# daxiongpro/EPNet

Measured on AMD Instinct MI355X. Metric: SA-stack points/sec per GPU (16384-pt KITTI scene) + % HBM roofline, higher is better.
Workload: dtype f32; 1 GPU; 256 x 16384-pt kitti scenes per GPU per step through the 4-level SA op stack (4 samplings [FPS + centre gather; levels 2-4 nested in level 1 where tie-free] + 8 ball_query + 8 fused groupings [xyz - centre ; features]), pyramid 16384>4096>1024>256>64, radii [[.1,.5],[.5,1],[1,2],[2,4]], nsample [16,32], C=0/96/256/512, HIP-graph launch; levels=4, scenes_per_gpu=256, software_pipelined=True, pipeline_stages=2, parallelism=scene-parallel x1

## Files before the change

epnet_amd/csrc/ball_query.hip:

```cpp

#include "common.h"
#include "dpp.h"
#include "spatial.h"

namespace epnet {

constexpr int kBqTile = 2048;
constexpr int kBqThreads = 256;

template <int CPW>
__global__ __launch_bounds__(kBqThreads) void ball_query_kernel(int n, int m, float radius2, int nsample,
                                                                const float *__restrict__ new_xyz,
                                                                const float *__restrict__ xyz,
                                                                int *__restrict__ idx) {
    __shared__ float tile[kBqTile * 3];
    const int lane = threadIdx.x & 63, wave = threadIdx.x >> 6;
    const int bs = blockIdx.y;
    xyz += (size_t)bs * n * 3;
    new_xyz += (size_t)bs * m * 3;
    idx += (size_t)bs * m * nsample;

    const int c0 = (blockIdx.x * (kBqThreads / 64) + wave) * CPW;
    float cx[CPW], cy[CPW], cz[CPW];
    int cnt[CPW], first[CPW];
#pragma unroll
    for (int i = 0; i < CPW; ++i) {
        const int ci = c0 + i;
        const bool ok = ci < m;
        cx[i] = ok ? new_xyz[ci * 3 + 0] : 0.f;
        cy[i] = ok ? new_xyz[ci * 3 + 1] : 0.f;
        cz[i] = ok ? new_xyz[ci * 3 + 2] : 0.f;
        cnt[i] = ok ? 0 : nsample;
        first[i] = 0;
    }

    for (int t0 = 0; t0 < n; t0 += kBqTile) {
        const int tn = min(kBqTile, n - t0);
        for (int e = threadIdx.x; e < tn * 3; e += kBqThreads) tile[e] = xyz[(size_t)t0 * 3 + e];
        __syncthreads();

        bool wave_done = true;
#pragma unroll
        for (int i = 0; i < CPW; ++i) wave_done = wave_done && (cnt[i] >= nsample);

        if (!wave_done) {
            for (int p0 = 0; p0 < tn; p0 += 64) {
                const int p = p0 + lane;
                const bool valid = p < tn;
                const float x = valid ? tile[p * 3 + 0] : 0.f;
                const float y = valid ? tile[p * 3 + 1] : 0.f;
                const float z = valid ? tile[p * 3 + 2] : 0.f;
                bool all_full = true;
#pragma unroll
                for (int i = 0; i < CPW; ++i) {
                    if (cnt[i] < nsample) {
                        const float dx = cx[i] - x, dy = cy[i] - y, dz = cz[i] - z;
                        const float d2 = dx * dx + dy * dy + dz * dz;
                        const bool hit = valid && (d2 < radius2);
                        const unsigned long long mask = __ballot(hit);
                        if (mask) {
                            const int pos = cnt[i] + popc_below(mask);
                            if (hit && pos < nsample) idx[(size_t)(c0 + i) * nsample + pos] = t0 + p;
                            if (cnt[i] == 0) first[i] = t0 + p0 + (int)__builtin_ctzll(mask);
                            cnt[i] += (int)__popcll(mask);
                        }
                        all_full = all_full && (cnt[i] >= nsample);
                    }
                }
                if (all_full) {
                    wave_done = true;
                    break;
                }
            }
        }
        if (__syncthreads_and(wave_done ? 1 : 0)) break;
    }

#pragma unroll
    for (int i = 0; i < CPW; ++i) {
        const int ci = c0 + i;
        if (ci < m && cnt[i] < nsample) {
            const int fill = cnt[i] > 0 ? first[i] : 0;
            for (int l = cnt[i] + lane; l < nsample; l += 64) idx[(size_t)ci * nsample + l] = fill;
        }
    }
}



#ifdef EPNET_BQ_STATS
__device__ unsigned long long g_bq_stats[16];
#endif
#ifdef EPNET_IX_STATS
__device__ unsigned long long g_ix_stats[8];
#define EPNET_IX_STAMP(var) const unsigned long long var = __builtin_amdgcn_s_memtime()
#else
#define EPNET_IX_STAMP(var)
#endif

template <int kIxThreads, int BITS>
__global__ __launch_bounds__(kIxThreads) void bq_index_kernel(int n, int np, const float *__restrict__ xyz,
                                                              float4 *__restrict__ sorted, float *__restrict__ boxes,
                                                              float *__restrict__ qboxes, int n_src = 0,
                                                              const int *__restrict__ src_idx = nullptr,
                                                              float *__restrict__ gathered = nullptr) {
    constexpr int kCells = 1 << BITS;
    extern __shared__ int s_hist[];
    __shared__ float s_box[6][16];
    __shared__ int s_part[16];
    const int q = threadIdx.x, lane = q & 63, wave = q >> 6;
    __builtin_amdgcn_s_setprio(3);
    xyz += (size_t)blockIdx.x * (src_idx ? n_src : n) * 3;
    if (src_idx) {
        src_idx += (size_t)blockIdx.x * n;
        gathered += (size_t)blockIdx.x * n * 3;
    }
    sorted += (size_t)blockIdx.x * np;
    boxes += (size_t)blockIdx.x * (np / 64) * 6;
    constexpr int per = kCells / kIxThreads;
    constexpr int per_shift = per == 16 ? 4 : per == 8 ? 3 : per == 4 ? 2 : -1;
    static_assert(per_shift > 0, "scan layout");
    constexpr int kIxPerThread = 16;
    const bool in_regs = n <= kIxThreads * kIxPerThread;
    float px[kIxPerThread], py[kIxPerThread], pz[kIxPerThread];
    float lo[3], ext[3];
    EPNET_IX_STAMP(t_0);
    if (in_regs) {
        float mn[3] = {3.4e38f, 3.4e38f, 3.4e38f}, mx[3] = {-3.4e38f, -3.4e38f, -3.4e38f};
        int row[kIxPerThread];
#pragma unroll
        for (int i = 0; i < kIxPerThread; ++i) {
            const int k = q + i * kIxThreads;
            const int kk = k < n ? k : 0;
            row[i] = src_idx ? src_idx[kk] : kk;
        }
#pragma unroll
        for (int i = 0; i < kIxPerThread; ++i) {
            px[i] = xyz[row[i] * 3 + 0];
            py[i] = xyz[row[i] * 3 + 1];
            pz[i] = xyz[row[i] * 3 + 2];
        }
        if (src_idx) {
#pragma unroll
            for (int i = 0; i < kIxPerThread; ++i) {
                const int k = q + i * kIxThreads;
                if (k < n) {
                    gathered[k * 3 + 0] = px[i];
                    gathered[k * 3 + 1] = py[i];
                    gathered[k * 3 + 2] = pz[i];
                }
            }
        }
#pragma unroll
        for (int i = 0; i < kIxPerThread; ++i) {
            const bool ok = q + i * kIxThreads < n;
            mn[0] = fminf(mn[0], ok ? px[i] : 3.4e38f); mx[0] = fmaxf(mx[0], ok ? px[i] : -3.4e38f);
            mn[1] = fminf(mn[1], ok ? py[i] : 3.4e38f); mx[1] = fmaxf(mx[1], ok ? py[i] : -3.4e38f);
            mn[2] = fminf(mn[2], ok ? pz[i] : 3.4e38f); mx[2] = fmaxf(mx[2], ok ? pz[i] : -3.4e38f);
        }
#pragma unroll
        for (int a = 0; a < 3; ++a) {
            const float l = wave_minf_all(mn[a]), h = wave_maxf_all(mx[a]);
            if (lane == 0) {
                s_box[a][wave] = l;
                s_box[3 + a][wave] = h;
            }
        }
        __syncthreads();
#pragma unroll
        for (int a = 0; a < 3; ++a) {
            float l = s_box[a][0], h = s_box[3 + a][0];
            for (int w = 1; w < kIxThreads / 64; ++w) {
                l = fminf(l, s_box[a][w]);
                h = fmaxf(h, s_box[3 + a][w]);
            }
            lo[a] = l;
            ext[a] = h - l;
        }
    } else {
        block_bbox3(xyz, n, s_box, lo, ext);
    }
    const CellGrid g = make_cell_grid(lo, ext, BITS);
    EPNET_IX_STAMP(t_1);
    for (int i = q; i < kCells + kCells / per + 64; i += kIxThreads) s_hist[i] = 0;
    __syncthreads();
    EPNET_IX_STAMP(t_2);
    int code[kIxPerThread], rank[kIxPerThread];
    if (in_regs) {
#pragma unroll
        for (int i = 0; i < kIxPerThread; ++i) code[i] = hist_at((int)cell_code(g, px[i], py[i], pz[i]), per_shift);
#pragma unroll
        for (int i = 0; i < kIxPerThread; ++i)
            rank[i] = atomicAdd(&s_hist[q + i * kIxThreads < n ? code[i] : kCells + kCells / per + lane], 1);
    } else {
        for (int k = q; k < n; k += kIxThreads)
            atomicAdd(&s_hist[hist_at((int)cell_code(g, xyz[k * 3 + 0], xyz[k * 3 + 1], xyz[k * 3 + 2]), per_shift)], 1);
    }
    __syncthreads();
    EPNET_IX_STAMP(t_3);
    int sum = 0;
    for (int i = 0; i < per; ++i) sum += s_hist[hist_at(q * per + i, per_shift)];
    const int incl = wave_inclusive_scan(sum);
    if (lane == 63) s_part[wave] = incl;
    __syncthreads();
    int base = incl - sum;
    for (int w = 0; w < wave; ++w) base += s_part[w];
    for (int i = 0; i < per; ++i) {
        const int at = hist_at(q * per + i, per_shift);
        const int c = s_hist[at];
        s_hist[at] = base;
        base += c;
    }
    __syncthreads();
    EPNET_IX_STAMP(t_4);
    auto bucket_box = [&](int p, const float4 v) {
        const bool real = p < n;
        const float cx_ = canonical(v.x), cy_ = canonical(v.y), cz_ = canonical(v.z);
        float mnx = real ? cx_ : 3.4e38f, mxx = real ? cx_ : -3.4e38f, mny = real ? cy_ : 3.4e38f, mxy = real ? cy_ : -3.4e38f,
              mnz = real ? cz_ : 3.4e38f, mxz = real ? cz_ : -3.4e38f;
        wave_box(mnx, mxx, mny, mxy, mnz, mxz);
        if (lane == 0) {
            float *bx = boxes + (p >> 6) * 6;
            const bool any = mnx <= mxx;
            bx[0] = any ? mnx : 3.0e38f; bx[1] = any ? mxx : 3.0e38f;
            bx[2] = any ? mny : 3.0e38f; bx[3] = any ? mxy : 3.0e38f;
            bx[4] = any ? mnz : 3.0e38f; bx[5] = any ? mxz : 3.0e38f;
        }
    };
    const bool staged = in_regs && (np & 255) == 0;
    if (staged) {
        float4 *s_stage = reinterpret_cast<float4 *>(s_hist + kCells + kCells / per + 64);
        int pos[kIxPerThread];
#pragma unroll
        for (int i = 0; i < kIxPerThread; ++i) pos[i] = s_hist[code[i]] + rank[i];
        const int quarter = kIxThreads == 256 ? min(np >> 2, 512) : np >> 2;
        for (int h = 0; h * quarter < np; ++h) {
            const int base = h * quarter, len = min(quarter, np - base);
            for (int p = q; p < len; p += kIxThreads)
                if (base + p >= n) s_stage[p] = make_float4(3.0e38f, 3.0e38f, 3.0e38f, __int_as_float(-1));
#pragma unroll
            for (int i = 0; i < kIxPerThread; ++i) {
                const int k = q + i * kIxThreads;
                if (k < n && (unsigned)(pos[i] - base) < (unsigned)quarter)
                    s_stage[pos[i] - base] = make_float4(px[i], py[i], pz[i], __int_as_float(k));
            }
            __syncthreads();
            for (int p = q; p < len; p += kIxThreads) {
                const float4 v = s_stage[p];
                sorted[base + p] = v;
                bucket_box(base + p, v);
            }
            __syncthreads();
        }
    } else {
        if (in_regs) {
#pragma unroll
            for (int i = 0; i < kIxPerThread; ++i) {
                const int k = q + i * kIxThreads;
                if (k < n) sorted[s_hist[code[i]] + rank[i]] = make_float4(px[i], py[i], pz[i], __int_as_float(k));
            }
        } else {
            for (int k = q; k < n; k += kIxThreads) {
                const float x = xyz[k * 3 + 0], y = xyz[k * 3 + 1], z = xyz[k * 3 + 2];
                const int pos = atomicAdd(&s_hist[hist_at((int)cell_code(g, x, y, z), per_shift)], 1);
                sorted[pos] = make_float4(x, y, z, __int_as_float(k));
            }
        }
        for (int p = n + q; p < np; p += kIxThreads)
            sorted[p] = make_float4(3.0e38f, 3.0e38f, 3.0e38f, __int_as_float(-1));
        __threadfence_block();
        __syncthreads();
        for (int p = q; p < np; p += kIxThreads) bucket_box(p, sorted[p]);
    }
#ifdef EPNET_IX_STATS
    {
        EPNET_IX_STAMP(t_6);
        if (q == 0) {
            atomicAdd(&g_ix_stats[0], t_1 - t_0); atomicAdd(&g_ix_stats[1], t_2 - t_1); atomicAdd(&g_ix_stats[2], t_3 - t_2);
            atomicAdd(&g_ix_stats[3], t_4 - t_3); atomicAdd(&g_ix_stats[4], t_6 - t_4);
            atomicAdd(&g_ix_stats[7], 1ull);
        }
    }
#endif
    if (!qboxes) return;
    qboxes += (size_t)blockIdx.x * (np / 256) * 6;
    __threadfence_block();
    __syncthreads();
    for (int g = q; g < np / 256; g += kIxThreads) {
        float mn[3] = {3.4e38f, 3.4e38f, 3.4e38f}, mx[3] = {-3.4e38f, -3.4e38f, -3.4e38f};
        for (int k = 0; k < 4; ++k) {
            const float *bx = boxes + (g * 4 + k) * 6;
            if (bx[0] < 3.0e38f)
#pragma unroll
                for (int a = 0; a < 3; ++a) {
                    mn[a] = fminf(mn[a], bx[2 * a]);
                    mx[a] = fmaxf(mx[a], bx[2 * a + 1]);
                }
        }
        const bool any = mn[0] <= mx[0];
#pragma unroll
        for (int a = 0; a < 3; ++a) {
            qboxes[g * 6 + 2 * a] = any ? mn[a] : 3.0e38f;
            qboxes[g * 6 + 2 * a + 1] = any ? mx[a] : 3.0e38f;
        }
    }
}

constexpr int kQThreads = 256;

__device__ __forceinline__ bool box_near(const float *__restrict__ bx, float cx, float cy, float cz, float radius2) {
    const float2 bxx = *reinterpret_cast<const float2 *>(bx), byy = *reinterpret_cast<const float2 *>(bx + 2),
                 bzz = *reinterpret_cast<const float2 *>(bx + 4);
    const float px = __builtin_amdgcn_fmed3f(cx, bxx.x, bxx.y), py = __builtin_amdgcn_fmed3f(cy, byy.x, byy.y),
                pz = __builtin_amdgcn_fmed3f(cz, bzz.x, bzz.y);
    const float dx = cx - px, dy = cy - py, dz = cz - pz;
    return (dx * dx + dy * dy + dz * dz) < radius2;
}


template <int DPL, typename F>
__device__ __forceinline__ void bq_walk(int lane, int np, float r2, float cx, float cy, float cz,
                                        const float4 *__restrict__ sorted, const float *__restrict__ boxes,
                                        const float *__restrict__ qboxes, int *quads, F &&visit) {
    auto scan_buckets = [&](unsigned long long cand, auto &&bucket_of) {
        while (cand) {
            float4 p[4];
            int nb = 0;
#pragma unroll
            for (int k = 0; k < 4; ++k)
                if (cand) {
                    const int bb = bucket_of((int)__builtin_ctzll(cand));
                    cand &= cand - 1ull;
                    p[k] = sorted[(bb << 6) + lane];
                    nb = k + 1;
                }
#pragma unroll
            for (int k = 0; k < 4; ++k)
                if (k < nb) {
                    const float dx = cx - p[k].x, dy = cy - p[k].y, dz = cz - p[k].z;
                    visit(p[k], dx * dx + dy * dy + dz * dz);
                }
        }
    };
    if constexpr (DPL <= 2) {
        const bool bnear = lane < (np >> 6) && box_near(boxes + lane * 6, cx, cy, cz, r2);
        scan_buckets(__ballot(bnear), [](int l) { return l; });
    } else {
        const int nq = np >> 8;
        for (int q0 = 0; q0 < nq; q0 += 64) {
            const int qd = q0 + lane;
            const bool qnear = qd < nq && box_near(qboxes + qd * 6, cx, cy, cz, r2);
            const unsigned long long qmask = __ballot(qnear);
            if (!qmask) continue;
            const int nqc = (int)__popcll(qmask);
            if (qnear) quads[popc_below(qmask)] = qd;
            __builtin_amdgcn_wave_barrier();
            for (int s0 = 0; s0 < nqc; s0 += 16) {
                const int slot = s0 + (lane >> 2);
                int bid = 0;
                bool bnear = false;
                if (slot < nqc) {
                    bid = quads[slot] * 4 + (lane & 3);
                    bnear = box_near(boxes + bid * 6, cx, cy, cz, r2);
                }
                scan_buckets(__ballot(bnear), [&](int l) { return __builtin_amdgcn_readlane(bid, l); });
            }
            __builtin_amdgcn_wave_barrier();
        }
    }
}

__device__ __forceinline__ void bq_emit_list(int lane, const int *hits, int cnt, int nsample, int *__restrict__ out) {
    __builtin_amdgcn_wave_barrier();
    const int mine = lane < cnt ? hits[lane] : 0x7fffffff;
    int rank = 0;
    for (int j = 0; j < cnt; ++j) rank += __builtin_amdgcn_readlane(mine, j) < mine ? 1 : 0;
    if (lane < cnt && rank < nsample) out[rank] = mine;
    int first = 0;
    if (cnt) first = __builtin_amdgcn_readlane(mine, (int)__builtin_ctzll(__ballot(lane < cnt && rank == 0)));
    for (int l = cnt + lane; l < nsample; l += 64) out[l] = first;
}

template <int RM>
__device__ __forceinline__ int bq_select_smallest(int lane, int *hits, int cnt, int nsample, int np) {
    __builtin_amdgcn_wave_barrier();
    int key[RM];
#pragma unroll
    for (int r = 0; r < RM; ++r) key[r] = (r * 64 < cnt && r * 64 + lane < cnt) ? hits[r * 64 + lane] : 0x7fffffff;
    int lo = 0, hi = np;
    while (hi - lo > 1) {
        const int mid = (lo + hi) >> 1;
        int c = 0;
#pragma unroll
        for (int r = 0; r < RM; ++r)
            if (r * 64 < cnt) c += (int)__popcll(__ballot(key[r] < mid));
        if (c >= nsample) hi = mid;
        else lo = mid;
    }
    __builtin_amdgcn_wave_barrier();
    int base = 0;
#pragma unroll
    for (int r = 0; r < RM; ++r)
        if (r * 64 < cnt) {
            const bool sel = key[r] < hi;
            const unsigned long long sm = __ballot(sel);
            if (sel) hits[base + popc_below(sm)] = key[r];
            base += (int)__popcll(sm);
        }
    return hi;
}

template <int DPL>
__device__ __forceinline__ void bq_bitmap_search(int lane, int np, float r2, int nsample, float cx, float cy, float cz,
                                                 const float4 *__restrict__ sorted, const float *__restrict__ boxes,
                                                 const float *__restrict__ qboxes, int *__restrict__ out, unsigned *bits,
                                                 int *quads) {
#pragma unroll
    for (int w = 0; w < DPL; ++w) bits[lane * DPL + w] = 0u;
    __builtin_amdgcn_wave_barrier();
    bq_walk<DPL>(lane, np, r2, cx, cy, cz, sorted, boxes, qboxes, quads, [&](const float4 &p, float d2) {
        if (d2 < r2) {
            const int k = __float_as_int(p.w);
            atomicOr(&bits[k >> 5], 1u << (k & 31));
        }
    });
    __builtin_amdgcn_wave_barrier();
    int bc = 0;
#pragma unroll 8
    for (int i = 0; i < DPL; ++i) bc += __popc(bits[lane * DPL + i]);
    const int incl = wave_inclusive_scan(bc);
    const int total = __builtin_amdgcn_readlane(incl, 63);
    int pos = incl - bc;
    int mine_first = 0x7fffffff;
    if (bc > 0 && (pos < nsample || pos == 0)) {
        for (int i = 0; i < DPL; ++i) {
            unsigned ww = bits[lane * DPL + i];
            if (ww && mine_first == 0x7fffffff) mine_first = (lane * DPL + i) * 32 + (int)__builtin_ctz(ww);
            while (ww && pos < nsample) {
                const int bit = (int)__builtin_ctz(ww);
                ww &= ww - 1u;
                out[pos++] = (lane * DPL + i) * 32 + bit;
            }
            if (pos >= nsample) break;
        }
    }
    const unsigned long long have = __ballot(bc > 0);
    int first = 0;
    if (have) first = __builtin_amdgcn_readlane(mine_first, (int)__builtin_ctzll(have));
    for (int l = total + lane; l < nsample; l += 64) out[l] = first;
}

template <int K>
struct BqScales {
    float r2[K];
    int nsample[K];
    int *idx[K];
};

template <int DPL, int K>
__global__ __launch_bounds__(kQThreads) void bq_query_kernel(int np, int m, BqScales<K> sc,
                                                             const float *__restrict__ new_xyz,
                                                             const float4 *__restrict__ sorted,
                                                             const float *__restrict__ boxes,
                                                             const float *__restrict__ qboxes,
                                                             const float4 *__restrict__ order, int npc) {
    __shared__ unsigned s_bits[kQThreads / 64][64 * DPL];
    __shared__ int s_quads[kQThreads / 64][64];
    __shared__ int s_hits[kQThreads / 64][K][64];
    const int lane = threadIdx.x & 63, wave = threadIdx.x >> 6;
    int wg_x, bs;
    xcd_scene_map(wg_x, bs);
    int ci = wg_x * (kQThreads / 64) + wave;
    if (ci >= m) return;
    sorted += (size_t)bs * np;
    boxes += (size_t)bs * (np / 64) * 6;
    qboxes += (size_t)bs * (np / 256) * 6;
    float cx, cy, cz;
    if (order) {
        const float4 e = order[(size_t)bs * npc + ci];
        ci = __float_as_int(e.w);
        cx = e.x; cy = e.y; cz = e.z;
    } else {
        const float *c = new_xyz + ((size_t)bs * m + ci) * 3;
        cx = c[0]; cy = c[1]; cz = c[2];
    }
    float r2max = sc.r2[0];
#pragma unroll
    for (int k = 1; k < K; ++k) r2max = fmaxf(r2max, sc.r2[k]);
    int cnt[K];
#pragma unroll
    for (int k = 0; k < K; ++k) cnt[k] = 0;
    bq_walk<DPL>(lane, np, r2max, cx, cy, cz, sorted, boxes, qboxes, s_quads[wave], [&](const float4 &p, float d2) {
        if (!__ballot(d2 < r2max)) return;
#pragma unroll
        for (int k = 0; k < K; ++k) {
            const bool hit = d2 < sc.r2[k];
            const unsigned long long hm = __ballot(hit);
            if (hm) {
                const int pos = cnt[k] + popc_below(hm);
                if (hit && pos < 64) s_hits[wave][k][pos] = __float_as_int(p.w);
                cnt[k] += (int)__popcll(hm);
            }
        }
    });
#pragma unroll
    for (int k = 0; k < K; ++k) {
        int *out = sc.idx[k] + ((size_t)bs * m + ci) * sc.nsample[k];
        if (cnt[k] <= 64)
            bq_emit_list(lane, s_hits[wave][k], cnt[k], sc.nsample[k], out);
        else
            bq_bitmap_search<DPL>(lane, np, sc.r2[k], sc.nsample[k], cx, cy, cz, sorted, boxes, qboxes, out, s_bits[wave],
                                  s_quads[wave]);
    }
}

template <int DPL, int K, bool kStream>
__global__ __launch_bounds__(kQThreads) void bq_query2_kernel(int np, int m, BqScales<K> sc,
                                                              const float *__restrict__ new_xyz,
                                                              const float4 *__restrict__ sorted,
                                                              const float *__restrict__ boxes,
                                                              const float *__restrict__ qboxes,
                                                              const float4 *__restrict__ order, int npc) {
    constexpr int kRowsPerStep = 2;
    constexpr int CAP = kStream ? (K == 1 ? 512 : 256) : 64, kStepAppends = kRowsPerStep * 64;
    static_assert(CAP % 64 == 0, "the lists are selected and emitted in whole waves");
    static_assert(!kStream || CAP - kStepAppends >= 64,
                  "a cut list keeps nsample <= 64 entries (the launcher streams for nsample <= 64 only) and must take a step's appends");
    constexpr int kBitWords = kStream ? 0 : 64 * DPL;
    __shared__ unsigned s_pool[kQThreads / 64][kBitWords + 2 * K * CAP];
    __shared__ int s_quads[kQThreads / 64][2][64];
    const int lane = threadIdx.x & 63, wave = threadIdx.x >> 6;
    int wg_x, bs;
    xcd_scene_map(wg_x, bs);
    const int ci0 = (wg_x * (kQThreads / 64) + wave) * 2;
    if (ci0 >= m) return;
    const bool two = ci0 + 1 < m;
    sorted += (size_t)bs * np;
    boxes += (size_t)bs * (np / 64) * 6;
    qboxes += (size_t)bs * (np / 256) * 6;
    float ax, ay, az, bx_, by_, bz_;
    int out0 = ci0, out1 = ci0 + 1;
    if (order) {
        const float4 e0 = order[(size_t)bs * npc + ci0], e1 = order[(size_t)bs * npc + ci0 + (two ? 1 : 0)];
        ax = e0.x; ay = e0.y; az = e0.z;
        bx_ = e1.x; by_ = e1.y; bz_ = e1.z;
        out0 = __float_as_int(e0.w);
        out1 = __float_as_int(e1.w);
    } else {
        const float *c0 = new_xyz + ((size_t)bs * m + ci0) * 3;
        const float *c1 = two ? c0 + 3 : c0;
        ax = c0[0]; ay = c0[1]; az = c0[2];
        bx_ = c1[0]; by_ = c1[1]; bz_ = c1[2];
    }
    const int half = lane >> 5;
    const float hx = half ? bx_ : ax, hy = half ? by_ : ay, hz = half ? bz_ : az;
    float r2max = sc.r2[0];
#pragma unroll
    for (int k = 1; k < K; ++k) r2max = fmaxf(r2max, sc.r2[k]);
    int cnt[2][K];
    int below[2][K];
#pragma unroll
    for (int e = 0; e < 2; ++e)
#pragma unroll
        for (int k = 0; k < K; ++k) {
            cnt[e][k] = 0;
            below[e][k] = 0x7fffffff;
        }
    int *hits_of = reinterpret_cast<int *>(s_pool[wave]) + kBitWords;
#ifdef EPNET_BQ_STATS
    const unsigned long long st_0 = __builtin_amdgcn_s_memtime();
    unsigned st_rows = 0;
    bool st_sel = false, st_again = false;
#endif

    auto visit = [&](int e, const float4 &p) {
#ifdef EPNET_BQ_STATS
        ++st_rows;
#endif
        const float cx = e ? bx_ : ax, cy = e ? by_ : ay, cz = e ? bz_ : az;
        const float dx = cx - p.x, dy = cy - p.y, dz = cz - p.z;
        const float d2 = dx * dx + dy * dy + dz * dz;
        if (!__ballot(d2 < r2max)) return;
#pragma unroll
        for (int k = 0; k < K; ++k) {
            const bool hit = d2 < sc.r2[k] && (!kStream || __float_as_int(p.w) < below[e][k]);
            const unsigned long long hm = __ballot(hit);
            if (hm) {
                const int pos = cnt[e][k] + popc_below(hm);
                if (hit && pos < CAP) hits_of[(e * K + k) * CAP + pos] = __float_as_int(p.w);
                cnt[e][k] += (int)__popcll(hm);
            }
        }
    };
    auto make_room = [&]() {
        if constexpr (kStream) {
#pragma unroll
            for (int e = 0; e < 2; ++e)
#pragma unroll
                for (int k = 0; k < K; ++k)
                    if (cnt[e][k] > CAP - kStepAppends) {
                        below[e][k] = bq_select_smallest<CAP / 64>(lane, hits_of + (e * K + k) * CAP, cnt[e][k], sc.nsample[k], np);
                        cnt[e][k] = sc.nsample[k];
#ifdef EPNET_BQ_STATS
                        st_sel = true;
#endif
                    }
        }
    };
    auto scan_pairs = [&](unsigned long long cand0, unsigned long long cand1, auto &&bucket_of) {
        static_assert(kRowsPerStep == 2, "the step below loads two rows of each centre");
        while (cand0 | cand1) {
            make_room();
            float4 p0 = make_float4(0.f, 0.f, 0.f, 0.f), p1 = p0, p2 = p0, p3 = p0;
            const bool h0 = cand0 != 0ull, h1 = cand1 != 0ull;
            if (h0) { p0 = sorted[(bucket_of(0, (int)__builtin_ctzll(cand0)) << 6) + lane]; cand0 &= cand0 - 1ull; }
            if (h1) { p1 = sorted[(bucket_of(1, (int)__builtin_ctzll(cand1)) << 6) + lane]; cand1 &= cand1 - 1ull; }
            const bool h2 = cand0 != 0ull, h3 = cand1 != 0ull;
            if (h2) { p2 = sorted[(bucket_of(0, (int)__builtin_ctzll(cand0)) << 6) + lane]; cand0 &= cand0 - 1ull; }
            if (h3) { p3 = sorted[(bucket_of(1, (int)__builtin_ctzll(cand1)) << 6) + lane]; cand1 &= cand1 - 1ull; }
            if (h0) visit(0, p0);
            if (h1) visit(1, p1);
            if (h2) visit(0, p2);
            if (h3) visit(1, p3);
        }
    };
    if constexpr (DPL <= 2) {
        bool n0 = false, n1 = false;
        if (lane < (np >> 6)) {
            n0 = box_near(boxes + lane * 6, ax, ay, az, r2max);
            n1 = box_near(boxes + lane * 6, bx_, by_, bz_, r2max);
        }
        scan_pairs(__ballot(n0), __ballot(n1), [](int, int bit) { return bit; });
    } else {
        const int nq = np >> 8;
        for (int q0 = 0; q0 < nq; q0 += 64) {
            const int qd = q0 + lane;
            bool n0 = false, n1 = false;
            if (qd < nq) {
                n0 = box_near(qboxes + qd * 6, ax, ay, az, r2max);
                n1 = box_near(qboxes + qd * 6, bx_, by_, bz_, r2max);
            }
            const unsigned long long qm0 = __ballot(n0), qm1 = __ballot(n1);
            if (!(qm0 | qm1)) continue;
            const int nq0 = (int)__popcll(qm0), nq1 = (int)__popcll(qm1);
            if (n0) s_quads[wave][0][popc_below(qm0)] = qd;
            if (n1) s_quads[wave][1][popc_below(qm1)] = qd;
            __builtin_amdgcn_wave_barrier();
            const int nmine = half ? nq1 : nq0;
            for (int s0 = 0; s0 < max(nq0, nq1); s0 += 8) {
                const int slot = s0 + ((lane & 31) >> 2);
                int bid = 0;
                bool bnear = false;
                if (slot < nmine) {
                    bid = s_quads[wave][half][slot] * 4 + (lane & 3);
                    bnear = box_near(boxes + bid * 6, hx, hy, hz, r2max);
                }
                const unsigned long long cand = __ballot(bnear);
                scan_pairs(cand & 0xFFFFFFFFull, cand >> 32,
                           [&](int e, int bit) { return __builtin_amdgcn_readlane(bid, bit + 32 * e); });
            }
            __builtin_amdgcn_wave_barrier();
        }
    }
#ifdef EPNET_BQ_STATS
    const unsigned long long st_1 = __builtin_amdgcn_s_memtime();
#endif
#pragma unroll
    for (int e = 0; e < 2; ++e) {
        if (e == 1 && !two) break;
        const float cx = e ? bx_ : ax, cy = e ? by_ : ay, cz = e ? bz_ : az;
#pragma unroll
        for (int k = 0; k < K; ++k) {
            int *out = sc.idx[k] + ((size_t)bs * m + (e ? out1 : out0)) * sc.nsample[k];
            int *hits = hits_of + (e * K + k) * CAP;
            if constexpr (kStream) {
                if (cnt[e][k] > 64) {
                    bq_select_smallest<CAP / 64>(lane, hits, cnt[e][k], sc.nsample[k], np);
                    cnt[e][k] = sc.nsample[k];
#ifdef EPNET_BQ_STATS
                    st_sel = true;
#endif
                }
                bq_emit_list(lane, hits, cnt[e][k], sc.nsample[k], out);
            } else {
                if (cnt[e][k] <= 64) {
                    bq_emit_list(lane, hits, cnt[e][k], sc.nsample[k], out);
                } else {
#ifdef EPNET_BQ_STATS
                    st_again = true;
#endif
                    bq_bitmap_search<DPL>(lane, np, sc.r2[k], sc.nsample[k], cx, cy, cz, sorted, boxes, qboxes, out, s_pool[wave],
                                          s_quads[wave][0]);
                }
            }
        }
    }
#ifdef EPNET_BQ_STATS
    {
        const unsigned long long st_3 = __builtin_amdgcn_s_memtime();
        if (lane == 0) {
            const int o = st_again ? 8 : (st_sel ? 4 : 0);
            atomicAdd(&g_bq_stats[o + 0], 1ull);
            atomicAdd(&g_bq_stats[o + 1], st_1 - st_0);
            atomicAdd(&g_bq_stats[o + 2], st_3 - st_1);
            atomicAdd(&g_bq_stats[o + 3], (unsigned long long)st_rows);
            atomicMax(&g_bq_stats[12], st_3 - st_0);
        }
    }
#endif
}

}

using namespace epnet;

extern "C" int epnet_ball_query(int b, int n, int m, float radius, int nsample, const float *new_xyz,
                                const float *xyz, int *idx, epnet_stream_t stream) {
    EPNET_REQUIRE(b >= 0 && n >= 0 && m >= 0 && nsample >= 0);
    if (b == 0 || m == 0 || nsample == 0) return EPNET_OK;
    EPNET_REQUIRE(new_xyz && xyz && idx);
    EPNET_REQUIRE(b <= 65535);
    const float radius2 = radius * radius;
    hipStream_t s = (hipStream_t)stream;
    constexpr int waves = kBqThreads / 64;
    if ((long long)m * b >= 8192) {
        dim3 grid(div_up(m, waves * 2), b);
        hipLaunchKernelGGL(ball_query_kernel<2>, grid, dim3(kBqThreads), 0, s, n, m, radius2, nsample, new_xyz, xyz, idx);
    } else {
        dim3 grid(div_up(m, waves), b);
        hipLaunchKernelGGL(ball_query_kernel<1>, grid, dim3(kBqThreads), 0, s, n, m, radius2, nsample, new_xyz, xyz, idx);
    }
    return check_launch("ball_query");
}


int epnet::spatial_index_launch(int b, int n, int np, const float *xyz, float4 *sorted, float *boxes, float *qboxes,
                                hipStream_t s, int n_src, const int *src_idx, float *gathered) {
    if (n <= 4096) {
        constexpr int T = 256, cells = 1 << 12;
        const size_t stage = (np & 255) == 0 ? (size_t)(np / 4 < 512 ? np / 4 : 512) * sizeof(float4) : 0;
        hipLaunchKernelGGL((bq_index_kernel<T, 12>), dim3(b), dim3(T), (size_t)(cells + cells / (cells / T) + 64) * sizeof(int) + stage, s,
                           n, np, xyz, sorted, boxes, qboxes, n_src, src_idx, gathered);
    } else {
        constexpr int T = 1024, cells = 1 << 14;
        const size_t stage = (n <= T * 16 && (np & 255) == 0) ? (size_t)(np / 4) * sizeof(float4) : 0;
        hipLaunchKernelGGL((bq_index_kernel<T, 14>), dim3(b), dim3(T), (size_t)(cells + cells / (cells / T) + 64) * sizeof(int) + stage, s,
                           n, np, xyz, sorted, boxes, qboxes, n_src, src_idx, gathered);
    }
    return check_launch("spatial index");
}

template <int K>
static int bq_query_launch(int b, int np, int m, const BqScales<K> &sc, const float *new_xyz, const float4 *sorted,
                           hipStream_t s, const float4 *order = nullptr, int npc = 0) {
    const float *boxes = (const float *)(sorted + (size_t)b * np);
    const float *qboxes = boxes + (size_t)b * (np / 64) * 6;
    const int pair_force = tuning(kBqPair);
    const bool pair = pair_force >= 0 ? pair_force != 0 : (long long)b * m >= 65536;
    if (pair) {
        dim3 grid(div_up(div_up(m, 2), kQThreads / 64), b);
        const int stream_force = tuning(kBqStream);
        bool stream = stream_force >= 0 ? stream_force != 0 : np > 16384;
        for (int k = 0; k < K; ++k) stream = stream && sc.nsample[k] <= 64;
#define EPNET_BQ2(D_)                                                                                                                   \
    do {                                                                                                                                \
        if (stream)                                                                                                                     \
            hipLaunchKernelGGL((bq_query2_kernel<D_, K, true>), grid, dim3(kQThreads), 0, s, np, m, sc, new_xyz, sorted, boxes, qboxes,   \
                               order, npc);                                                                                             \
        else                                                                                                                            \
            hipLaunchKernelGGL((bq_query2_kernel<D_, K, false>), grid, dim3(kQThreads), 0, s, np, m, sc, new_xyz, sorted, boxes,         \
                               qboxes, order, npc);                                                                                     \
    } while (0)
        switch (np / 2048) {
            case 1: EPNET_BQ2(1); break;
            case 2: EPNET_BQ2(2); break;
            case 4: EPNET_BQ2(4); break;
            case 8: EPNET_BQ2(8); break;
            case 16: EPNET_BQ2(16); break;
            default: EPNET_BQ2(32); break;
        }
#undef EPNET_BQ2
        return check_launch("ball_query query");
    }
    dim3 grid(div_up(m, kQThreads / 64), b);
#define EPNET_BQ(D_) hipLaunchKernelGGL((bq_query_kernel<D_, K>), grid, dim3(kQThreads), 0, s, np, m, sc, new_xyz, sorted, boxes, qboxes, order, npc)
    switch (np / 2048) {
        case 1: EPNET_BQ(1); break;
        case 2: EPNET_BQ(2); break;
        case 4: EPNET_BQ(4); break;
        case 8: EPNET_BQ(8); break;
        case 16: EPNET_BQ(16); break;
        default: EPNET_BQ(32); break;
    }
#undef EPNET_BQ
    return check_launch("ball_query query");
}

extern "C" size_t epnet_scene_index_bytes(int b, int n) { return scene_index_bytes(b, n); }

extern "C" int epnet_scene_index_build(int b, int n, const float *xyz, void *index, size_t index_bytes,
                                       epnet_stream_t stream) {
    const size_t need = scene_index_bytes(b, n);
    EPNET_REQUIRE(need != 0 && xyz && index);
    if (index_bytes < need) return EPNET_ENOMEM;
    if (((uintptr_t)index & 15) != 0) return EPNET_EINVAL;
    EPNET_REQUIRE(b <= 65535);
    const int np = scene_index_np(n);
    float4 *sorted = (float4 *)index;
    float *boxes = (float *)(sorted + (size_t)b * np);
    return spatial_index_launch(b, n, np, xyz, sorted, boxes, boxes + (size_t)b * (np / 64) * 6, (hipStream_t)stream);
}

extern "C" int epnet_scene_index_build_gathered(int b, int n_src, int n, const float *xyz_src, const int *idx, float *gathered,
                                                void *index, size_t index_bytes, epnet_stream_t stream) {
    const size_t need = scene_index_bytes(b, n);
    EPNET_REQUIRE(need != 0 && n <= 16384 && n_src >= 1 && xyz_src && idx && gathered && index);
    if (index_bytes < need) return EPNET_ENOMEM;
    if (((uintptr_t)index & 15) != 0) return EPNET_EINVAL;
    EPNET_REQUIRE(b <= 65535);
    const int np = scene_index_np(n);
    float4 *sorted = (float4 *)index;
    float *boxes = (float *)(sorted + (size_t)b * np);
    return spatial_index_launch(b, n, np, xyz_src, sorted, boxes, boxes + (size_t)b * (np / 64) * 6, (hipStream_t)stream, n_src, idx,
                                gathered);
}

extern "C" int epnet_ball_query_indexed(int b, int n, int m, float radius, int nsample, const float *new_xyz,
                                        const float *xyz, const void *index, size_t index_bytes, int *idx,
                                        epnet_stream_t stream) {
    const size_t need = scene_index_bytes(b, n);
    if (need == 0 || !index || nsample <= 0 || m <= 0)
        return epnet_ball_query(b, n, m, radius, nsample, new_xyz, xyz, idx, stream);
    EPNET_REQUIRE(new_xyz && idx);
    if (index_bytes < need) return EPNET_ENOMEM;
    EPNET_REQUIRE(b <= 65535);
    const int np = scene_index_np(n);
    BqScales<1> sc;
    sc.r2[0] = radius * radius;
    sc.nsample[0] = nsample;
    sc.idx[0] = idx;
    return bq_query_launch<1>(b, np, m, sc, new_xyz, (const float4 *)index, (hipStream_t)stream);
}

extern "C" int epnet_ball_query_indexed_multi(int b, int n, int m, int nscales, const float *radii, const int *nsamples,
                                              const float *new_xyz, const float *xyz, const void *index,
                                              size_t index_bytes, int *const *idx, epnet_stream_t stream) {
    EPNET_REQUIRE(nscales >= 0 && (nscales == 0 || (radii && nsamples && idx)));
    const size_t need = scene_index_bytes(b, n);
    bool fused = nscales == 2 && need != 0 && index && m > 0 && nsamples[0] > 0 && nsamples[1] > 0;
    if (!fused) {
        for (int k = 0; k < nscales; ++k) {
            const int rc = epnet_ball_query_indexed(b, n, m, radii[k], nsamples[k], new_xyz, xyz, index, index_bytes, idx[k], stream);
            if (rc) return rc;
        }
        return EPNET_OK;
    }
    EPNET_REQUIRE(new_xyz && idx[0] && idx[1]);
    if (index_bytes < need) return EPNET_ENOMEM;
    EPNET_REQUIRE(b <= 65535);
    BqScales<2> sc;
    for (int k = 0; k < 2; ++k) {
        sc.r2[k] = radii[k] * radii[k];
        sc.nsample[k] = nsamples[k];
        sc.idx[k] = idx[k];
    }
    return bq_query_launch<2>(b, scene_index_np(n), m, sc, new_xyz, (const float4 *)index, (hipStream_t)stream);
}

extern "C" int epnet_ball_query_ordered(int b, int n, int m, int nscales, const float *radii, const int *nsamples,
                                        const float *new_xyz, const float *xyz, const void *index, size_t index_bytes,
                                        const void *centre_index, size_t centre_index_bytes, int *const *idx,
                                        epnet_stream_t stream) {
    EPNET_REQUIRE(nscales >= 0 && (nscales == 0 || (radii && nsamples && idx)));
    const size_t need = scene_index_bytes(b, n), need_c = scene_index_bytes(b, m);
    bool ordered = (nscales == 1 || nscales == 2) && need != 0 && need_c != 0 && index && centre_index && m > 0;
    for (int k = 0; ordered && k < nscales; ++k) ordered = nsamples[k] > 0 && idx[k] != nullptr;
    const int force = tuning(kBqOrdered);
    if (force >= 0 ? force == 0 : n <= 16384) ordered = false;
    if (!ordered) return epnet_ball_query_indexed_multi(b, n, m, nscales, radii, nsamples, new_xyz, xyz, index, index_bytes, idx, stream);
    if (index_bytes < need || centre_index_bytes < need_c) return EPNET_ENOMEM;
    EPNET_REQUIRE(b <= 65535);
    const int np = scene_index_np(n), npc = scene_index_np(m);
    if (nscales == 1) {
        BqScales<1> sc;
        sc.r2[0] = radii[0] * radii[0];
        sc.nsample[0] = nsamples[0];
        sc.idx[0] = idx[0];
        return bq_query_launch<1>(b, np, m, sc, new_xyz, (const float4 *)index, (hipStream_t)stream, (const float4 *)centre_index, npc);
    }
    BqScales<2> sc;
    for (int k = 0; k < 2; ++k) {
        sc.r2[k] = radii[k] * radii[k];
        sc.nsample[k] = nsamples[k];
        sc.idx[k] = idx[k];
    }
    return bq_query_launch<2>(b, np, m, sc, new_xyz, (const float4 *)index, (hipStream_t)stream, (const float4 *)centre_index, npc);
}

extern "C" size_t epnet_ball_query_workspace_bytes(int b, int n, int m) {
    if (n < 1024 || m <= 0) return 0;
    return scene_index_bytes(b, n);
}

extern "C" int epnet_ball_query_ws(int b, int n, int m, float radius, int nsample, const float *new_xyz,
                                   const float *xyz, int *idx, void *workspace, size_t workspace_bytes,
                                   epnet_stream_t stream) {
    const size_t need = epnet_ball_query_workspace_bytes(b, n, m);
    if (need == 0 || nsample <= 0) return epnet_ball_query(b, n, m, radius, nsample, new_xyz, xyz, idx, stream);
    EPNET_REQUIRE(new_xyz && xyz && idx && workspace);
    int rc = epnet_scene_index_build(b, n, xyz, workspace, workspace_bytes, stream);
    if (rc) return rc;
    return epnet_ball_query_indexed(b, n, m, radius, nsample, new_xyz, xyz, workspace, workspace_bytes, idx, stream);
}

#ifdef EPNET_BQ_STATS
extern "C" int epnet_debug_bq_stats(unsigned long long *host16) {
    (void)hipMemcpyFromSymbol(host16, HIP_SYMBOL(epnet::g_bq_stats), sizeof(unsigned long long) * 16);
    unsigned long long zero[16] = {0};
    (void)hipMemcpyToSymbol(HIP_SYMBOL(epnet::g_bq_stats), zero, sizeof(zero));
    return 0;
}
#endif
#ifdef EPNET_IX_STATS
extern "C" int epnet_debug_ix_stats(unsigned long long *host8) {
    (void)hipMemcpyFromSymbol(host8, HIP_SYMBOL(epnet::g_ix_stats), sizeof(unsigned long long) * 8);
    unsigned long long zero[8] = {0};
    (void)hipMemcpyToSymbol(HIP_SYMBOL(epnet::g_ix_stats), zero, sizeof(zero));
    return 0;
}
#endif
```

Before: 1.434 billion points/s.

## Share one hit list across nested ball-query radii in the paired query kernel

For two-scale ball queries, the paired query kernel now records one hit list per centre at the larger radius. Each hit is tagged with a bit marking whether it also lies inside the smaller radius, and both outputs are emitted from that single list, including a paired emit path for short lists. A variant specialised to nsample 16/32 is added, along with scalarised (readfirstlane) centre coordinates and scene mapping, clamped quad-box loads and an explicit waitcnt in the row-scan loop. The aim is to halve the per-hit list appends and ballots. The trade-off is extra code complexity, and the overflow fallback now runs two bitmap searches.

```diff
diff --git a/epnet_amd/csrc/ball_query.hip b/epnet_amd/csrc/ball_query.hip
--- a/epnet_amd/csrc/ball_query.hip
+++ b/epnet_amd/csrc/ball_query.hip
@@ -381,6 +381,84 @@
     for (int l = cnt + lane; l < nsample; l += 64) out[l] = first;
 }
 
+
+__device__ __forceinline__ void bq_emit_shared(int lane, const int *hits, int cnt, int ns_big, int ns_small, int *__restrict__ out_big,
+                                               int *__restrict__ out_small) {
+    __builtin_amdgcn_wave_barrier();
+    const bool valid = lane < cnt;
+    const int mine = valid ? hits[lane] : 0x7fffffff;
+    int rank = 0, rin = 0;
+    for (int j = 0; j < cnt; ++j) {
+        const int v = __builtin_amdgcn_readlane(mine, j);
+        rank += v < mine ? 1 : 0;
+        rin += v < mine ? (v & 1) : 0;
+    }
+    const bool inner = valid && (mine & 1);
+    if (valid && rank < ns_big) out_big[rank] = mine >> 1;
+    if (inner && rin < ns_small) out_small[rin] = mine >> 1;
+    int first = 0;
+    if (cnt) first = __builtin_amdgcn_readlane(mine, (int)__builtin_ctzll(__ballot(valid && rank == 0))) >> 1;
+    for (int l = cnt + lane; l < ns_big; l += 64) out_big[l] = first;
+    const unsigned long long im = __ballot(inner);
+    const int cin = (int)__popcll(im);
+    first = 0;
+    if (cin) first = __builtin_amdgcn_readlane(mine, (int)__builtin_ctzll(__ballot(inner && rin == 0))) >> 1;
+    for (int l = cin + lane; l < ns_small; l += 64) out_small[l] = first;
+}
+
+template <int NS>
+__device__ __forceinline__ void bq_store_rows(int lane, bool two, const int *ord, int c0, int c1, int ns_rt, int *__restrict__ row0,
+                                              int *__restrict__ row1) {
+    const int ns = NS ? NS : ns_rt;
+    if (NS == 16 && lane >= 32) return;
+    const int e = NS == 16 ? lane >> 4 : lane >> 5, s = NS == 16 ? lane & 15 : lane & 31;
+    const int c = e ? c1 : c0;
+    int v = ord[e * 32 + (s < c ? s : 0)];
+    v = c ? v : 0;
+    if (e == 0) {
+        if (s < ns) row0[s] = v;
+    } else if (two) {
+        if (s < ns) row1[s] = v;
+    }
+    if (NS == 0 && ns > 32 && (e == 0 || two)) {
+        int *row = e ? row1 : row0;
+        const int first = c ? ord[e * 32] : 0;
+        for (int l = s + 32; l < ns; l += 32) row[l] = first;
+    }
+}
+
+template <int NSB, int NSS>
+__device__ __forceinline__ void bq_emit_pair(int lane, bool two, int *lists, int c0, int c1, int ns_big, int ns_small,
+                                             int *__restrict__ big0, int *__restrict__ big1, int *__restrict__ small0,
+                                             int *__restrict__ small1) {
+    const int half = lane >> 5, sl = lane & 31;
+    const int c = half ? c1 : c0;
+    int *raw = lists + half * 64;
+    const bool valid = sl < c;
+    __builtin_amdgcn_wave_barrier();
+    int mine = raw[sl];
+    if (!valid) {
+        mine = 0x7fffffff;
+        raw[sl] = mine;
+    }
+    __builtin_amdgcn_wave_barrier();
+    int rank = 0, rin = 0;
+    const int nmax = max(c0, c1);
+#pragma unroll 1
+    for (int j = 0; j < nmax; j += 4) {
+        const int4 v = *reinterpret_cast<const int4 *>(raw + j);
+        rank += (v.x < mine ? 1 : 0) + (v.y < mine ? 1 : 0) + (v.z < mine ? 1 : 0) + (v.w < mine ? 1 : 0);
+        rin += (v.x < mine ? v.x & 1 : 0) + (v.y < mine ? v.y & 1 : 0) + (v.z < mine ? v.z & 1 : 0) + (v.w < mine ? v.w & 1 : 0);
+    }
+    const bool inner = valid && (mine & 1);
+    if (valid) lists[128 + half * 32 + rank] = mine >> 1;
+    if (inner) lists[192 + half * 32 + rin] = mine >> 1;
+    const unsigned long long im = __ballot(inner);
+    __builtin_amdgcn_wave_barrier();
+    bq_store_rows<NSB>(lane, two, lists + 128, c0, c1, ns_big, big0, big1);
+    bq_store_rows<NSS>(lane, two, lists + 192, (int)__popc((unsigned)im), (int)__popc((unsigned)(im >> 32)), ns_small, small0, small1);
+}
+
 template <int RM>
 __device__ __forceinline__ int bq_select_smallest(int lane, int *hits, int cnt, int nsample, int np) {
     __builtin_amdgcn_wave_barrier();
@@ -433,6 +511,7 @@
     int pos = incl - bc;
     int mine_first = 0x7fffffff;
     if (bc > 0 && (pos < nsample || pos == 0)) {
+#pragma unroll 1
         for (int i = 0; i < DPL; ++i) {
             unsigned ww = bits[lane * DPL + i];
             if (ww && mine_first == 0x7fffffff) mine_first = (lane * DPL + i) * 32 + (int)__builtin_ctz(ww);
@@ -514,7 +593,24 @@
     }
 }
 
-template <int DPL, int K, bool kStream>
+__device__ __forceinline__ void xcd_scene_map_uniform(int &wg_x, int &bs) {
+#ifndef EPNET_NO_XCD_MAP
+    const int gx = (int)gridDim.x;
+    if ((gx & (gx - 1)) == 0) {
+        const int nwg = gx * (int)gridDim.y, orig = (int)blockIdx.y * gx + (int)blockIdx.x;
+        const int xcd = orig & 7, qq = nwg >> 3, rr = nwg & 7;
+        const int wgid = (xcd < rr ? xcd * (qq + 1) : rr * (qq + 1) + (xcd - rr) * qq) + (orig >> 3);
+        bs = wgid >> __builtin_ctz(gx);
+        wg_x = wgid & (gx - 1);
+        return;
+    }
+#endif
+    xcd_scene_map(wg_x, bs);
+    wg_x = __builtin_amdgcn_readfirstlane(wg_x);
+    bs = __builtin_amdgcn_readfirstlane(bs);
+}
+
+template <int DPL, int K, bool kStream, bool kSpec = false>
 __global__ __launch_bounds__(kQThreads) void bq_query2_kernel(int np, int m, BqScales<K> sc,
                                                               const float *__restrict__ new_xyz,
                                                               const float4 *__restrict__ sorted,
@@ -527,11 +623,13 @@
     static_assert(!kStream || CAP - kStepAppends >= 64,
                   "a cut list keeps nsample <= 64 entries (the launcher streams for nsample <= 64 only) and must take a step's appends");
     constexpr int kBitWords = kStream ? 0 : 64 * DPL;
-    __shared__ unsigned s_pool[kQThreads / 64][kBitWords + 2 * K * CAP];
+    constexpr bool kShared = K == 2 && !kStream;
+    static_assert(!kSpec || kShared, "the compile-time pair is one of the shared-list kernel");
+    __shared__ __attribute__((aligned(16))) unsigned s_pool[kQThreads / 64][kBitWords + 2 * K * CAP];
     __shared__ int s_quads[kQThreads / 64][2][64];
     const int lane = threadIdx.x & 63, wave = threadIdx.x >> 6;
     int wg_x, bs;
-    xcd_scene_map(wg_x, bs);
+    xcd_scene_map_uniform(wg_x, bs);
     const int ci0 = (wg_x * (kQThreads / 64) + wave) * 2;
     if (ci0 >= m) return;
     const bool two = ci0 + 1 < m;
@@ -552,11 +650,19 @@
         ax = c0[0]; ay = c0[1]; az = c0[2];
         bx_ = c1[0]; by_ = c1[1]; bz_ = c1[2];
     }
+    auto uniform = [](float v) { return __int_as_float(__builtin_amdgcn_readfirstlane(__float_as_int(v))); };
+    ax = uniform(ax); ay = uniform(ay); az = uniform(az);
+    bx_ = uniform(bx_); by_ = uniform(by_); bz_ = uniform(bz_);
+    out0 = __builtin_amdgcn_readfirstlane(out0);
+    out1 = __builtin_amdgcn_readfirstlane(out1);
     const int half = lane >> 5;
     const float hx = half ? bx_ : ax, hy = half ? by_ : ay, hz = half ? bz_ : az;
     float r2max = sc.r2[0];
 #pragma unroll
     for (int k = 1; k < K; ++k) r2max = fmaxf(r2max, sc.r2[k]);
+    const bool big1 = kSpec || (kShared && (sc.r2[K - 1] >= sc.r2[0] || sc.r2[0] != sc.r2[0]));
+    const float r2small = kShared ? (big1 ? sc.r2[0] : sc.r2[K - 1]) : r2max;
+    if constexpr (kShared) r2max = big1 ? sc.r2[K - 1] : sc.r2[0];
     int cnt[2][K];
     int below[2][K];
 #pragma unroll
@@ -580,6 +686,15 @@
         const float cx = e ? bx_ : ax, cy = e ? by_ : ay, cz = e ? bz_ : az;
         const float dx = cx - p.x, dy = cy - p.y, dz = cz - p.z;
         const float d2 = dx * dx + dy * dy + dz * dz;
+        if constexpr (kShared) {
+            const bool hit = d2 < r2max;
+            const unsigned long long hm = __ballot(hit);
+            if (!hm) return;
+            const int pos = cnt[e][0] + popc_below(hm);
+            if (hit && pos < 64) hits_of[e * 64 + pos] = (__float_as_int(p.w) << 1) | (d2 < r2small ? 1 : 0);
+            cnt[e][0] += (int)__popcll(hm);
+            return;
+        }
         if (!__ballot(d2 < r2max)) return;
 #pragma unroll
         for (int k = 0; k < K; ++k) {
@@ -607,21 +722,23 @@
                     }
         }
     };
+    auto row_of = [&](int bucket) { return (sorted + ((size_t)(unsigned)bucket << 6))[(unsigned)lane]; };
     auto scan_pairs = [&](unsigned long long cand0, unsigned long long cand1, auto &&bucket_of) {
         static_assert(kRowsPerStep == 2, "the step below loads two rows of each centre");
         while (cand0 | cand1) {
             make_room();
-            float4 p0 = make_float4(0.f, 0.f, 0.f, 0.f), p1 = p0, p2 = p0, p3 = p0;
+            float4 p0, p1, p2, p3;
             const bool h0 = cand0 != 0ull, h1 = cand1 != 0ull;
-            if (h0) { p0 = sorted[(bucket_of(0, (int)__builtin_ctzll(cand0)) << 6) + lane]; cand0 &= cand0 - 1ull; }
-            if (h1) { p1 = sorted[(bucket_of(1, (int)__builtin_ctzll(cand1)) << 6) + lane]; cand1 &= cand1 - 1ull; }
+            if (h0) { p0 = row_of(bucket_of(0, (int)__builtin_ctzll(cand0))); cand0 &= cand0 - 1ull; }
+            if (h1) { p1 = row_of(bucket_of(1, (int)__builtin_ctzll(cand1))); cand1 &= cand1 - 1ull; }
             const bool h2 = cand0 != 0ull, h3 = cand1 != 0ull;
-            if (h2) { p2 = sorted[(bucket_of(0, (int)__builtin_ctzll(cand0)) << 6) + lane]; cand0 &= cand0 - 1ull; }
-            if (h3) { p3 = sorted[(bucket_of(1, (int)__builtin_ctzll(cand1)) << 6) + lane]; cand1 &= cand1 - 1ull; }
+            if (h2) { p2 = row_of(bucket_of(0, (int)__builtin_ctzll(cand0))); cand0 &= cand0 - 1ull; }
+            if (h3) { p3 = row_of(bucket_of(1, (int)__builtin_ctzll(cand1))); cand1 &= cand1 - 1ull; }
             if (h0) visit(0, p0);
             if (h1) visit(1, p1);
             if (h2) visit(0, p2);
             if (h3) visit(1, p3);
+            __builtin_amdgcn_s_waitcnt(0x0F70);
         }
     };
     if constexpr (DPL <= 2) {
@@ -635,12 +752,9 @@
         const int nq = np >> 8;
         for (int q0 = 0; q0 < nq; q0 += 64) {
             const int qd = q0 + lane;
-            bool n0 = false, n1 = false;
-            if (qd < nq) {
-                n0 = box_near(qboxes + qd * 6, ax, ay, az, r2max);
-                n1 = box_near(qboxes + qd * 6, bx_, by_, bz_, r2max);
-            }
-            const unsigned long long qm0 = __ballot(n0), qm1 = __ballot(n1);
+            const float *qb = qboxes + __umul24(min(qd, nq - 1), 6);
+            const bool n0 = box_near(qb, ax, ay, az, r2max) && qd < nq, n1 = box_near(qb, bx_, by_, bz_, r2max) && qd < nq;
+            const unsigned long long qm0 = __builtin_amdgcn_ballot_w64(n0), qm1 = __builtin_amdgcn_ballot_w64(n1);
             if (!(qm0 | qm1)) continue;
             const int nq0 = (int)__popcll(qm0), nq1 = (int)__popcll(qm1);
             if (n0) s_quads[wave][0][popc_below(qm0)] = qd;
@@ -653,9 +767,9 @@
                 bool bnear = false;
                 if (slot < nmine) {
                     bid = s_quads[wave][half][slot] * 4 + (lane & 3);
-                    bnear = box_near(boxes + bid * 6, hx, hy, hz, r2max);
+                    bnear = box_near(boxes + __umul24(bid, 6), hx, hy, hz, r2max);
                 }
-                const unsigned long long cand = __ballot(bnear);
+                const unsigned long long cand = __builtin_amdgcn_ballot_w64(bnear);
                 scan_pairs(cand & 0xFFFFFFFFull, cand >> 32,
                            [&](int e, int bit) { return __builtin_amdgcn_readlane(bid, bit + 32 * e); });
             }
@@ -665,32 +779,62 @@
 #ifdef EPNET_BQ_STATS
     const unsigned long long st_1 = __builtin_amdgcn_s_memtime();
 #endif
-#pragma unroll
-    for (int e = 0; e < 2; ++e) {
-        if (e == 1 && !two) break;
-        const float cx = e ? bx_ : ax, cy = e ? by_ : ay, cz = e ? bz_ : az;
-#pragma unroll
-        for (int k = 0; k < K; ++k) {
-            int *out = sc.idx[k] + ((size_t)bs * m + (e ? out1 : out0)) * sc.nsample[k];
-            int *hits = hits_of + (e * K + k) * CAP;
-            if constexpr (kStream) {
-                if (cnt[e][k] > 64) {
-                    bq_select_smallest<CAP / 64>(lane, hits, cnt[e][k], sc.nsample[k], np);
-                    cnt[e][k] = sc.nsample[k];
-#ifdef EPNET_BQ_STATS
-                    st_sel = true;
-#endif
-                }
-                bq_emit_list(lane, hits, cnt[e][k], sc.nsample[k], out);
-            } else {
-                if (cnt[e][k] <= 64) {
-                    bq_emit_list(lane, hits, cnt[e][k], sc.nsample[k], out);
+    if constexpr (kShared) {
+        const int ns0 = kSpec ? 16 : sc.nsample[0], ns1 = kSpec ? 32 : sc.nsample[K - 1];
+        const int ns_big = big1 ? ns1 : ns0, ns_small = big1 ? ns0 : ns1;
+        int *idx_big = big1 ? sc.idx[K - 1] : sc.idx[0], *idx_small = big1 ? sc.idx[0] : sc.idx[K - 1];
+        const size_t row0 = (size_t)bs * m + out0, row1 = (size_t)bs * m + out1;
+        const int c0 = cnt[0][0], c1 = cnt[1][0];
+        if (c0 <= 32 && c1 <= 32) {
+            bq_emit_pair<kSpec ? 32 : 0, kSpec ? 16 : 0>(lane, two, hits_of, c0, c1, ns_big, ns_small, idx_big + row0 * ns_big,
+                                                         idx_big + row1 * ns_big, idx_small + row0 * ns_small, idx_small + row1 * ns_small);
+        } else {
+#pragma unroll
+            for (int e = 0; e < 2; ++e) {
+                if (e == 1 && !two) break;
+                const size_t row = e ? row1 : row0;
+                if (cnt[e][0] <= 64) {
+                    bq_emit_shared(lane, hits_of + e * 64, cnt[e][0], ns_big, ns_small, idx_big + row * ns_big, idx_small + row * ns_small);
                 } else {
 #ifdef EPNET_BQ_STATS
                     st_again = true;
 #endif
-                    bq_bitmap_search<DPL>(lane, np, sc.r2[k], sc.nsample[k], cx, cy, cz, sorted, boxes, qboxes, out, s_pool[wave],
+                    const float cx = e ? bx_ : ax, cy = e ? by_ : ay, cz = e ? bz_ : az;
+                    bq_bitmap_search<DPL>(lane, np, r2max, ns_big, cx, cy, cz, sorted, boxes, qboxes, idx_big + row * ns_big, s_pool[wave],
                                           s_quads[wave][0]);
+                    bq_bitmap_search<DPL>(lane, np, r2small, ns_small, cx, cy, cz, sorted, boxes, qboxes, idx_small + row * ns_small,
+                                          s_pool[wave], s_quads[wave][0]);
+                }
+            }
+        }
+    } else {
+#pragma unroll
+        for (int e = 0; e < 2; ++e) {
+            if (e == 1 && !two) break;
+            const float cx = e ? bx_ : ax, cy = e ? by_ : ay, cz = e ? bz_ : az;
+#pragma unroll
+            for (int k = 0; k < K; ++k) {
+                int *out = sc.idx[k] + ((size_t)bs * m + (e ? out1 : out0)) * sc.nsample[k];
+                int *hits = hits_of + (e * K + k) * CAP;
+                if constexpr (kStream) {
+                    if (cnt[e][k] > 64) {
+                        bq_select_smallest<CAP / 64>(lane, hits, cnt[e][k], sc.nsample[k], np);
+                        cnt[e][k] = sc.nsample[k];
+#ifdef EPNET_BQ_STATS
+                        st_sel = true;
+#endif
+                    }
+                    bq_emit_list(lane, hits, cnt[e][k], sc.nsample[k], out);
+                } else {
+                    if (cnt[e][k] <= 64) {
+                        bq_emit_list(lane, hits, cnt[e][k], sc.nsample[k], out);
+                    } else {
+#ifdef EPNET_BQ_STATS
+                        st_again = true;
+#endif
+                        bq_bitmap_search<DPL>(lane, np, sc.r2[k], sc.nsample[k], cx, cy, cz, sorted, boxes, qboxes, out, s_pool[wave],
+                                              s_quads[wave][0]);
+                    }
                 }
             }
         }
@@ -762,11 +906,15 @@
         const int stream_force = tuning(kBqStream);
         bool stream = stream_force >= 0 ? stream_force != 0 : np > 16384;
         for (int k = 0; k < K; ++k) stream = stream && sc.nsample[k] <= 64;
+        const bool spec = K == 2 && !stream && sc.nsample[0] == 16 && sc.nsample[K - 1] == 32 && sc.r2[0] <= sc.r2[K - 1];
 #define EPNET_BQ2(D_)                                                                                                                   \
     do {                                                                                                                                \
         if (stream)                                                                                                                     \
             hipLaunchKernelGGL((bq_query2_kernel<D_, K, true>), grid, dim3(kQThreads), 0, s, np, m, sc, new_xyz, sorted, boxes, qboxes,   \
                                order, npc);                                                                                             \
+        else if (spec)                                                                                                                  \
+            hipLaunchKernelGGL((bq_query2_kernel<D_, K, false, K == 2>), grid, dim3(kQThreads), 0, s, np, m, sc, new_xyz, sorted, boxes, \
+                               qboxes, order, npc);                                                                                     \
         else                                                                                                                            \
             hipLaunchKernelGGL((bq_query2_kernel<D_, K, false>), grid, dim3(kQThreads), 0, s, np, m, sc, new_xyz, sorted, boxes,         \
                                qboxes, order, npc);                                                                                     \
diff --git a/profiles/micro/step_tails.py b/profiles/micro/step_tails.py
--- /dev/null
+++ b/profiles/micro/step_tails.py
@@ -0,0 +1,28 @@
+import csv, statistics, sys
+rows = list(csv.DictReader(open(sys.argv[1])))
+skip = int(sys.argv[2]) if len(sys.argv) > 2 else 3
+rows.sort(key=lambda r: int(r["Start_Timestamp"]))
+name = lambda r: r["Kernel_Name"].replace("epnet::", "").replace("void ", "").split("(")[0]
+anchors = [i for i, r in enumerate(rows) if "fps_indexed_kernel<8, 32" in r["Kernel_Name"]]
+steps = []
+for a, b in zip(anchors[skip:-skip - 1], anchors[skip + 1:-skip]):
+    t0, t1 = int(rows[a]["Start_Timestamp"]), int(rows[b]["Start_Timestamp"])
+    fps_end = int(rows[a]["End_Timestamp"])
+    s_queue = rows[a]["Queue_Id"]
+    inside = [r for r in rows[a:b] if int(r["Start_Timestamp"]) < t1]
+    s_end = max(int(r["End_Timestamp"]) for r in inside if r["Queue_Id"] == s_queue)
+    g = [r for r in inside if r["Queue_Id"] != s_queue and "bq_index_kernel<1024" not in r["Kernel_Name"]]
+    g_end = max(int(r["End_Timestamp"]) for r in g if int(r["Start_Timestamp"]) > fps_end - 500000)
+    q1 = [r for r in g if "bq_query2_kernel<8" in r["Kernel_Name"]]
+    d = {"step": t1 - t0, "fps L1": fps_end - t0, "S tail (fps end -> S end)": s_end - fps_end, "S end": s_end - t0, "G end": g_end - t0}
+    if q1:
+        d["L1 query start - fps end"] = int(q1[0]["Start_Timestamp"]) - fps_end
+    for r in inside:
+        if int(r["Start_Timestamp"]) >= fps_end - 300000 and "gather_rows" not in r["Kernel_Name"]:
+            k = ("S " if r["Queue_Id"] == s_queue else "G ") + name(r)
+            d[k] = d.get(k, 0) + int(r["End_Timestamp"]) - int(r["Start_Timestamp"])
+    steps.append(d)
+print("%d steady steps" % len(steps))
+for k in steps[0]:
+    v = [s[k] / 1e6 for s in steps if k in s]
+    print("%-58s median %7.3f  min %7.3f  max %7.3f ms" % (k[:58], statistics.median(v), min(v), max(v)))
```

Result: faster. 1.468 billion points/s, median of 6 (+2.3%).
